# hmorimitsu/ptlflow

Measured on AMD Instinct MI355X. Metric: frame-pairs/sec, RAFT 32-iter 436x1024, higher is better.
Workload: dtype f32; 1 GPU; raft random-init (seeded), 436x1024 frame pairs, 32 iterations, fp32, batch 8/GPU, eval forward incl. encoders, mask head + convex upsample on every iteration as the reference; global_batch=8, parallelism=dp1 (independent replicas, no collectives)

## Files before the change

ptlflow_amd/csrc/pfk_wino.hip:

```cpp
#include "pfk_gemm.h"

using namespace pfkg;

namespace {

constexpr int WT = 32;
constexpr int WN = 64;
constexpr int WK = 8;
constexpr int UIMG = 16 * WN * WK;

typedef float f32x2 __attribute__((ext_vector_type(2)));
typedef __attribute__((address_space(3))) float lfloat;
typedef __attribute__((address_space(3))) f32x2 lf32x2;
typedef __attribute__((address_space(3))) f32x4 lf32x4;

struct WinoArgs {
  const float* src; int ld;
  unsigned src_bytes;
  int H, W;
  int tw, tpi;
  int ntiles;
  int nks;
  const float* weight; unsigned w_bytes;
  const float* bias;
  int cout;
  int ncb;
  int relu; float scale;
  float* out; int out_ld, out_coff;
  const float* res; int res_ld;
  int relu2;
};

__device__ __forceinline__ __amdgpu_buffer_rsrc_t rsrc_n(const void* p, unsigned bytes) {
  return __builtin_amdgcn_make_buffer_rsrc(const_cast<void*>(p), 0, (int)bytes, 0x00020000);
}

__device__ __forceinline__ void wino_load_v2(__amdgpu_buffer_rsrc_t rs, const unsigned (&voff)[16], int ks, int q, float (&d)[16]) {
  d[q] = __builtin_bit_cast(float, __builtin_amdgcn_raw_buffer_load_b32(rs, voff[q], ks * WK * 4, 0));
  d[q + 1] = __builtin_bit_cast(float, __builtin_amdgcn_raw_buffer_load_b32(rs, voff[q + 1], ks * WK * 4, 0));
}

__device__ __forceinline__ void wino_dma_u(__amdgpu_buffer_rsrc_t rw, lfloat* dst, unsigned wvoff, unsigned wk, int j) {
#if defined(__HIP_DEVICE_COMPILE__)
  __builtin_amdgcn_raw_ptr_buffer_load_lds(rw, (__attribute__((address_space(3))) void*)(dst + j * 1024), 16, wvoff, wk + j * 4096u, 0, 0);
#endif
}

__device__ __forceinline__ void wino_mfma(const lfloat* aV, const lfloat* aU, const lfloat* aU1, f32x4 (&acc)[16][2], bool more,
                                          __amdgpu_buffer_rsrc_t rw, lfloat* udst, unsigned wvoff, unsigned wk,
                                          __amdgpu_buffer_rsrc_t rs, const unsigned (&voff)[16], int ks, float (&d)[16]) {
  f32x2 va[2], u0[2], u1[2];
  va[0] = *(const lf32x2*)(aV);
  u0[0] = *(const lf32x2*)(aU);
  u1[0] = *(const lf32x2*)(aU1);
  __builtin_amdgcn_sched_barrier(0);
#pragma unroll
  for (int x = 0; x < 16; ++x) {
    const int c = x & 1, n = c ^ 1;
    if (x + 1 < 16) {
      va[n] = *(const lf32x2*)(aV + (x + 1) * WT * WK);
      u0[n] = *(const lf32x2*)(aU + (x + 1) * WN * WK);
      u1[n] = *(const lf32x2*)(aU1 + (x + 1) * WN * WK);
    }
    if (more) {
      if (x < 8) wino_dma_u(rw, udst, wvoff, wk, x);
      else wino_load_v2(rs, voff, ks, 2 * (x - 8), d);
    }
    __builtin_amdgcn_sched_barrier(0);
    acc[x][0] = __builtin_amdgcn_mfma_f32_16x16x4f32(va[c][0], u0[c][0], acc[x][0], 0, 0, 0);
    acc[x][1] = __builtin_amdgcn_mfma_f32_16x16x4f32(va[c][0], u1[c][0], acc[x][1], 0, 0, 0);
    acc[x][0] = __builtin_amdgcn_mfma_f32_16x16x4f32(va[c][1], u0[c][1], acc[x][0], 0, 0, 0);
    acc[x][1] = __builtin_amdgcn_mfma_f32_16x16x4f32(va[c][1], u1[c][1], acc[x][1], 0, 0, 0);
    __builtin_amdgcn_sched_barrier(0);
  }
}

template <bool RES>
__global__ __launch_bounds__(256, 2) void conv_gemm_wino_f32_kernel(const WinoArgs a) {
  __shared__ __attribute__((aligned(16))) float smem[2 * UIMG + 16 * WT * WK];
  lfloat* const sU = (lfloat*)smem;
  lfloat* const sV = sU + 2 * UIMG;

  const int tid = threadIdx.x, lane = tid & 63, wid = __builtin_amdgcn_readfirstlane(tid >> 6);
  const int cb = blockIdx.x % a.ncb;
  const int t0 = (blockIdx.x / a.ncb) * WT;

  const __amdgpu_buffer_rsrc_t rs = rsrc_n(a.src, a.src_bytes);
  const __amdgpu_buffer_rsrc_t rw = rsrc_n(a.weight, a.w_bytes);

  const int lt = tid >> 3, cc = tid & 7;
  unsigned voff[16];
  {
    const int g = t0 + lt;
    const bool tok = g < a.ntiles;
    const int b = g / a.tpi, r = g - b * a.tpi;
    const int ty = r / a.tw, tx = r - ty * a.tw;
#pragma unroll
    for (int i = 0; i < 4; ++i)
#pragma unroll
      for (int j = 0; j < 4; ++j) {
        const int y = 2 * ty - 1 + i, x = 2 * tx - 1 + j;
        const bool ok = tok && (unsigned)y < (unsigned)a.H && (unsigned)x < (unsigned)a.W;
        voff[i * 4 + j] = ok ? ((unsigned)((b * a.H + y) * a.W + x) * (unsigned)a.ld + (unsigned)cc) * 4u : OOB;
      }
  }
  const int vslot = ((cc & 3) * 2 + (cc >> 2)) ^ (((lt >> 2) & 3) * 2);
  lfloat* const vdst = sV + lt * WK + vslot;
  const unsigned wvoff = (unsigned)lane * 16u;
  const unsigned wbase = (unsigned)cb * (unsigned)a.nks * (UIMG * 4u) + (unsigned)wid * 1024u;
  lfloat* const udst = sU + wid * 256;

  float d[16];
  const int wt = wid & 1, wc = wid >> 1;
  const int rl = lane & 15, kq = lane >> 4;
  const lfloat* const aV = sV + (wt * 16 + rl) * WK + ((kq * 2) ^ (((rl >> 2) & 3) * 2));
  const lfloat* const aU = sU + (wc * 32 + rl) * WK + ((kq * 2) ^ (((rl >> 2) & 3) * 2));
  const lfloat* aU1 = aU + 16 * WK;
  asm volatile("" : "+v"(aU1));

  f32x4 acc[16][2];
#pragma unroll
  for (int x = 0; x < 16; ++x)
#pragma unroll
    for (int c = 0; c < 2; ++c) acc[x][c] = f32x4{0.f, 0.f, 0.f, 0.f};

#pragma unroll
  for (int j = 0; j < 8; ++j) {
    wino_dma_u(rw, udst, wvoff, wbase, j);
    wino_load_v2(rs, voff, 0, 2 * j, d);
  }
  for (int ks = 0; ks < a.nks; ++ks) {
    float t[16];
#pragma unroll
    for (int j = 0; j < 4; ++j) {
      t[0 * 4 + j] = d[0 * 4 + j] - d[2 * 4 + j];
      t[1 * 4 + j] = d[1 * 4 + j] + d[2 * 4 + j];
      t[2 * 4 + j] = d[2 * 4 + j] - d[1 * 4 + j];
      t[3 * 4 + j] = d[1 * 4 + j] - d[3 * 4 + j];
    }
#pragma unroll
    for (int i = 0; i < 4; ++i) {
      vdst[(i * 4 + 0) * WT * WK] = t[i * 4 + 0] - t[i * 4 + 2];
      vdst[(i * 4 + 1) * WT * WK] = t[i * 4 + 1] + t[i * 4 + 2];
      vdst[(i * 4 + 2) * WT * WK] = t[i * 4 + 2] - t[i * 4 + 1];
      vdst[(i * 4 + 3) * WT * WK] = t[i * 4 + 1] - t[i * 4 + 3];
    }
    asm volatile("s_waitcnt vmcnt(0) lgkmcnt(0)\n\ts_barrier" ::: "memory");
    const int ub = (ks & 1) * UIMG;
    wino_mfma(aV, aU + ub, aU1 + ub, acc, ks + 1 < a.nks, rw, udst + (UIMG - ub), wvoff, wbase + (unsigned)(ks + 1) * (UIMG * 4u), rs,
              voff, ks + 1, d);
    asm volatile("s_waitcnt lgkmcnt(0)\n\ts_barrier" ::: "memory");
  }

  typedef __attribute__((address_space(1))) float gfloat;
  gfloat* const outp = (gfloat*)a.out;
#pragma unroll
  for (int c = 0; c < 2; ++c) {
    const int n = cb * WN + wc * 32 + c * 16 + rl;
    const bool nok = n < a.cout;
    const float bias = (a.bias != nullptr && nok) ? a.bias[n] : 0.f;
#pragma unroll
    for (int r = 0; r < 4; ++r) {
      const int g = t0 + wt * 16 + kq * 4 + r;
      float m[16];
#pragma unroll
      for (int x = 0; x < 16; ++x) m[x] = acc[x][c][r];
      float s0[4], s1[4];
#pragma unroll
      for (int j = 0; j < 4; ++j) {
        s0[j] = m[0 * 4 + j] + m[1 * 4 + j] + m[2 * 4 + j];
        s1[j] = m[1 * 4 + j] - m[2 * 4 + j] - m[3 * 4 + j];
      }
      float y[4];
      y[0] = s0[0] + s0[1] + s0[2];
      y[1] = s0[1] - s0[2] - s0[3];
      y[2] = s1[0] + s1[1] + s1[2];
      y[3] = s1[1] - s1[2] - s1[3];
      if (!nok || g >= a.ntiles) continue;
      const int b = g / a.tpi, rr = g - b * a.tpi;
      const int ty = rr / a.tw, tx = rr - ty * a.tw;
#pragma unroll
      for (int e = 0; e < 4; ++e) {
        const int oy = 2 * ty + (e >> 1), ox = 2 * tx + (e & 1);
        if (oy >= a.H || ox >= a.W) continue;
        float v = y[e] + bias;
        if (a.relu) v = (v < 0.f) ? 0.f : v;
        v *= a.scale;
        const long long p = ((long long)b * a.H + oy) * a.W + ox;
        if constexpr (RES) {
          v = a.res[p * a.res_ld + n] + v;
          if (a.relu2) v = (v < 0.f) ? 0.f : v;
        }
        outp[p * a.out_ld + a.out_coff + n] = v;
      }
    }
  }
}

constexpr int WN1 = 128;
constexpr int VIMG1 = 8 * WT * WK;

struct Wino1dArgs {
  const float* src0; const float* src1;
  int ld0, ld1;
  unsigned bytes0, bytes1;
  int nks0, nks;
  int H, W;
  int L, nt;
  int ntiles;
  const float* weight; unsigned w_bytes;
  const float* bias;
  int cout, ncb;
  int relu; float scale;
  float* out; int out_ld, out_coff;
  const float* res; int res_ld;
  float* h; int h_ld;
  float* aux_z; float* aux_rh;
  int ch;
};

template <bool VERT>
__device__ __forceinline__ void wino1d_tile(const Wino1dArgs& a, int g, int& base, int& t) {
  if constexpr (VERT) {
    const int r = g / a.W, x = g - r * a.W, b = r / a.nt;
    t = r - b * a.nt;
    base = b * a.H * a.W + x;
  } else {
    const int line = g / a.nt;
    t = g - line * a.nt;
    base = line * a.W;
  }
}

__device__ __forceinline__ void wino1d_load_v(__amdgpu_buffer_rsrc_t rs0, __amdgpu_buffer_rsrc_t rs1, const unsigned (&voff0)[8],
                                              const unsigned (&voff1)[8], bool s1, int soff, int q, float (&d)[8]) {
  d[q] = s1 ? __builtin_bit_cast(float, __builtin_amdgcn_raw_buffer_load_b32(rs1, voff1[q], soff, 0))
            : __builtin_bit_cast(float, __builtin_amdgcn_raw_buffer_load_b32(rs0, voff0[q], soff, 0));
}

__device__ __forceinline__ void wino1d_mfma(const lfloat* aV, const lfloat* aU0, const lfloat* aU1, const lfloat* aU2, const lfloat* aU3,
                                            f32x4 (&acc)[8][4], bool more, __amdgpu_buffer_rsrc_t rw, lfloat* udst, unsigned wvoff,
                                            unsigned wk, __amdgpu_buffer_rsrc_t rs0, __amdgpu_buffer_rsrc_t rs1,
                                            const unsigned (&voff0)[8], const unsigned (&voff1)[8], bool s1, int soff, float (&d)[8]) {
  f32x2 va[2], u[2][4];
  va[0] = *(const lf32x2*)(aV);
  u[0][0] = *(const lf32x2*)(aU0);
  u[0][1] = *(const lf32x2*)(aU1);
  u[0][2] = *(const lf32x2*)(aU2);
  u[0][3] = *(const lf32x2*)(aU3);
  __builtin_amdgcn_sched_barrier(0);
#pragma unroll
  for (int x = 0; x < 8; ++x) {
    const int c = x & 1, n = c ^ 1;
    if (x + 1 < 8) {
      va[n] = *(const lf32x2*)(aV + (x + 1) * WT * WK);
      u[n][0] = *(const lf32x2*)(aU0 + (x + 1) * WN1 * WK);
      u[n][1] = *(const lf32x2*)(aU1 + (x + 1) * WN1 * WK);
      u[n][2] = *(const lf32x2*)(aU2 + (x + 1) * WN1 * WK);
      u[n][3] = *(const lf32x2*)(aU3 + (x + 1) * WN1 * WK);
    }
    if (more) {
      wino_dma_u(rw, udst, wvoff, wk, x);
      wino1d_load_v(rs0, rs1, voff0, voff1, s1, soff, x, d);
    }
    __builtin_amdgcn_sched_barrier(0);
#pragma unroll
    for (int s = 0; s < 2; ++s)
#pragma unroll
      for (int f = 0; f < 4; ++f) acc[x][f] = __builtin_amdgcn_mfma_f32_16x16x4f32(va[c][s], u[c][f][s], acc[x][f], 0, 0, 0);
    __builtin_amdgcn_sched_barrier(0);
  }
}

__device__ __forceinline__ void wino1d_at(const f32x4 (&acc)[8][4], int f, int r, float (&y)[4]) {
  const float p12 = acc[1][f][r] + acc[2][f][r], q12 = acc[1][f][r] - acc[2][f][r];
  const float p34 = acc[3][f][r] + acc[4][f][r], q34 = acc[3][f][r] - acc[4][f][r];
  const float p56 = acc[5][f][r] + acc[6][f][r], q56 = acc[5][f][r] - acc[6][f][r];
  y[0] = acc[0][f][r] + p12 + p34 + p56;
  y[1] = q12 + 2.f * q34 + 0.5f * q56;
// ... 209 lines not shown

int pfk_conv1d_wino_f32(const pfk_conv_desc* d, pfk_stream_t stream) {
  if (!d) return PFK_ERR_BAD_ARG;
  const bool vert = d->kh == 5 && d->kw == 1;
  if (!vert && !(d->kh == 1 && d->kw == 5)) return PFK_ERR_UNSUPPORTED;
  if (d->stride > 1 || d->num_src < 1 || d->num_src > 2 || d->relu_after_residual) return PFK_ERR_UNSUPPORTED;
  if (d->epilogue != PFK_EPI_LINEAR && d->epilogue != PFK_EPI_GRU_ZR && d->epilogue != PFK_EPI_GRU_Q) return PFK_ERR_UNSUPPORTED;
  if (d->cout_active > 0 && d->cout_active < d->cout) return PFK_ERR_UNSUPPORTED;
  if (d->epilogue == PFK_EPI_LINEAR && d->residual) return PFK_ERR_UNSUPPORTED;
  if (!d->weight || d->B <= 0 || d->H <= 0 || d->W <= 0 || d->cout <= 0) return PFK_ERR_BAD_ARG;
  const long long M = (long long)d->B * d->H * d->W;
  int ktot = 0;
  for (int i = 0; i < d->num_src; ++i) {
    const pfk_conv_src& s = d->src[i];
    if (!s.ptr || s.channels <= 0 || s.ld < s.channels) return PFK_ERR_BAD_ARG;
    if (s.channels & 7) return PFK_ERR_UNSUPPORTED;
    if (reinterpret_cast<uintptr_t>(s.ptr) & 3u) return PFK_ERR_ALIGNMENT;
    if (M * s.ld * 4 >= 0x7fffffffLL) return PFK_ERR_UNSUPPORTED;
    ktot += s.channels;
  }
  const int ch = d->epilogue == PFK_EPI_GRU_ZR ? d->cout / 2 : d->cout;
  if (d->epilogue == PFK_EPI_LINEAR) {
    if (!d->out || d->out_coff < 0 || d->out_ld < d->out_coff + d->cout) return PFK_ERR_BAD_ARG;
    if (reinterpret_cast<uintptr_t>(d->out) & 3u) return PFK_ERR_ALIGNMENT;
  } else {
    if (!d->h || !d->aux_z || d->h_ld < ch || (d->epilogue == PFK_EPI_GRU_ZR && (!d->aux_rh || (d->cout & 1))) || (ch & 3))
      return PFK_ERR_BAD_ARG;
    if (d->residual && d->residual_ld < d->cout) return PFK_ERR_BAD_ARG;
    if (!pfk_aligned16(d->h) || !pfk_aligned16(d->aux_z) || !pfk_aligned16(d->aux_rh) || !pfk_aligned16(d->residual) || (d->h_ld & 3) ||
        (d->residual && (d->residual_ld & 3)))
      return PFK_ERR_ALIGNMENT;
  }
  if (!pfk_aligned16(d->weight)) return PFK_ERR_ALIGNMENT;
  const long long wfloats = pfk_conv_wino1d_weight_floats(ktot, d->cout);
  if (wfloats * 4 >= 0x7fffffffLL) return PFK_ERR_UNSUPPORTED;
  Wino1dArgs a{};
  const pfk_conv_src& s0 = d->src[0];
  const pfk_conv_src& s1 = d->src[d->num_src - 1];
  a.src0 = s0.ptr; a.ld0 = s0.ld; a.bytes0 = (unsigned)(((M - 1) * s0.ld + s0.channels) * 4);
  a.src1 = s1.ptr; a.ld1 = s1.ld; a.bytes1 = (unsigned)(((M - 1) * s1.ld + s1.channels) * 4);
  a.nks0 = s0.channels / WK; a.nks = ktot / WK;
  a.H = d->H; a.W = d->W;
  a.L = vert ? d->H : d->W;
  a.nt = (a.L + 3) / 4;
  const long long ntiles = (long long)d->B * (vert ? d->W : d->H) * a.nt;
  a.ncb = (d->cout + WN1 - 1) / WN1;
  const long long nblk = (ntiles + WT - 1) / WT * a.ncb;
  if (nblk >= 0x7fffffffLL) return PFK_ERR_UNSUPPORTED;
  a.ntiles = (int)ntiles;
  a.weight = d->weight; a.w_bytes = (unsigned)(wfloats * 4);
  a.bias = d->bias;
  a.cout = d->cout;
  a.relu = d->relu ? 1 : 0; a.scale = d->scale;
  a.out = d->out; a.out_ld = d->out_ld; a.out_coff = d->out_coff;
  a.res = d->residual; a.res_ld = d->residual_ld;
  a.h = d->h; a.h_ld = d->h_ld; a.aux_z = d->aux_z; a.aux_rh = d->aux_rh; a.ch = ch;
  if (vert) wino1d_launch_epi<true>(a, d->epilogue, (unsigned)nblk, static_cast<hipStream_t>(stream));
  else wino1d_launch_epi<false>(a, d->epilogue, (unsigned)nblk, static_cast<hipStream_t>(stream));
  return pfk_launch_status();
}

long long pfk_conv_wino_weight_floats(int cin, int cout) {
  if (cin <= 0 || cout <= 0 || (cin & 31)) return PFK_ERR_BAD_ARG;
  return 16LL * cin * ((cout + WN - 1) / WN * WN);
}

static int wino_launch(const pfk_conv_desc* d, bool res, pfk_stream_t stream) {
  if (!d) return PFK_ERR_BAD_ARG;
  if (d->num_src != 1 || d->kh != 3 || d->kw != 3 || d->stride > 1 || d->epilogue != PFK_EPI_LINEAR)
    return PFK_ERR_UNSUPPORTED;
  if (!res && (d->residual || d->relu_after_residual)) return PFK_ERR_UNSUPPORTED;
  if (res && (!d->residual || d->residual_ld < d->cout || (reinterpret_cast<uintptr_t>(d->residual) & 3u))) return PFK_ERR_BAD_ARG;
  const pfk_conv_src& s = d->src[0];
  if (!s.ptr || !d->weight || !d->out || d->B <= 0 || d->H <= 0 || d->W <= 0 || d->cout <= 0 || s.channels <= 0 ||
      s.ld < s.channels || d->out_coff < 0 || d->out_ld < d->out_coff + d->cout)
    return PFK_ERR_BAD_ARG;
  if (s.channels & 31) return PFK_ERR_UNSUPPORTED;
  if (!pfk_aligned16(d->weight) || (reinterpret_cast<uintptr_t>(s.ptr) & 3u) || (reinterpret_cast<uintptr_t>(d->out) & 3u))
    return PFK_ERR_ALIGNMENT;
  const long long M = (long long)d->B * d->H * d->W;
  const long long src_bytes = ((M - 1) * s.ld + s.channels) * 4;
  const long long wfloats = pfk_conv_wino_weight_floats(s.channels, d->cout);
  if (M * s.ld * 4 >= 0x7fffffffLL || wfloats * 4 >= 0x7fffffffLL) return PFK_ERR_UNSUPPORTED;
  int ncb = (d->cout + WN - 1) / WN;
  if (d->cout_active > 0 && d->cout_active < d->cout) {
    if (d->cout_active & (WN - 1)) return PFK_ERR_UNSUPPORTED;
    ncb = d->cout_active / WN;
  }
  WinoArgs a{};
  a.src = s.ptr; a.ld = s.ld; a.src_bytes = (unsigned)src_bytes;
  a.H = d->H; a.W = d->W;
  a.tw = (d->W + 1) / 2;
  a.tpi = a.tw * ((d->H + 1) / 2);
  const long long ntiles = (long long)d->B * a.tpi;
  const long long nblk = (ntiles + WT - 1) / WT * ncb;
  if (nblk >= 0x7fffffffLL) return PFK_ERR_UNSUPPORTED;
  a.ntiles = (int)ntiles;
  a.nks = s.channels / WK;
  a.weight = d->weight; a.w_bytes = (unsigned)(wfloats * 4);
  a.bias = d->bias;
  a.cout = d->cout;
  a.ncb = ncb;
  a.relu = d->relu ? 1 : 0; a.scale = d->scale;
  a.out = d->out; a.out_ld = d->out_ld; a.out_coff = d->out_coff;
  if (res) {
    if (d->cout_active > 0 && d->cout_active < d->cout) return PFK_ERR_UNSUPPORTED;
    a.res = d->residual; a.res_ld = d->residual_ld; a.relu2 = d->relu_after_residual ? 1 : 0;
    hipLaunchKernelGGL(conv_gemm_wino_f32_kernel<true>, dim3((unsigned)nblk), dim3(256), 0, static_cast<hipStream_t>(stream), a);
  } else {
    hipLaunchKernelGGL(conv_gemm_wino_f32_kernel<false>, dim3((unsigned)nblk), dim3(256), 0, static_cast<hipStream_t>(stream), a);
  }
  return pfk_launch_status();
}

int pfk_conv2d_wino_f32(const pfk_conv_desc* d, pfk_stream_t stream) { return wino_launch(d, false, stream); }

int pfk_conv2d_wino_res_f32(const pfk_conv_desc* d, pfk_stream_t stream) { return wino_launch(d, true, stream); }



}
```

ptlflow_amd/update.py:

```python
from __future__ import annotations

from dataclasses import dataclass
from typing import Dict, List, Optional, Tuple

import torch

from . import load_native
from ._seam import WrappedModule, pixel_rows
from .packing import (pack_cin2_weight, pack_conv_weight, pack_flow_head_weight, pack_wino1d_weight, pack_wino_weight, permute_mask_head,
                      round_up, split_bf16_planes)

EPI_LINEAR, EPI_GRU_ZR, EPI_GRU_Q = 0, 1, 2


@dataclass(frozen=True)
class UpdateSpec:
    hidden: int
    context: int
    corr_channels: int
    c1: int
    c2: int
    f1: int
    f2: int
    enc_out: int
    gru_passes: Tuple[Tuple[int, int, str], ...]
    fh_hidden: int
    has_mask: bool
    aggregate: bool = False
    mask_channels: int = 576
    external_aggregate: bool = False

    @property
    def motion_channels(self) -> int:
        return self.enc_out + 2

    @property
    def x_channels(self) -> int:
        return self.context + self.motion_channels * (2 if self.aggregate else 1)

    @property
    def hx_channels(self) -> int:
        return round_up(self.hidden + self.x_channels, 4)


def basic_spec(corr_levels: int = 4, corr_radius: int = 4) -> UpdateSpec:
    return UpdateSpec(128, 128, corr_levels * (2 * corr_radius + 1) ** 2, 256, 192, 128, 64, 126,
                      ((1, 5, "1"), (5, 1, "2")), 256, True)


def gma_spec(corr_levels: int = 4, corr_radius: int = 4) -> UpdateSpec:
    return UpdateSpec(128, 128, corr_levels * (2 * corr_radius + 1) ** 2, 256, 192, 128, 64, 126,
                      ((1, 5, "1"), (5, 1, "2")), 256, True, True)


def ccmr_spec(corr_channels: int, mask_channels: int = 36) -> UpdateSpec:
    return UpdateSpec(128, 128, corr_channels, 256, 192, 128, 64, 126, ((1, 5, "1"), (5, 1, "2")), 256, True, True,
                      mask_channels, True)


def ms_raft_plus_spec(corr_channels: int, mask_channels: int = 36) -> UpdateSpec:
    return UpdateSpec(128, 128, corr_channels, 256, 192, 128, 64, 126, ((1, 5, "1"), (5, 1, "2")), 256, True, False,
                      mask_channels)


def small_spec(corr_levels: int = 4, corr_radius: int = 3) -> UpdateSpec:
    return UpdateSpec(96, 64, corr_levels * (2 * corr_radius + 1) ** 2, 96, 0, 64, 32, 80,
                      ((3, 3, ""),), 128, False)


WINO_MIN_WORK = 28160

WINO1D_MIN_PIXELS = 28160

SMALL_GRID_PIXELS = 28160

CONV_PRECISIONS = {"fp32": 0, "bf16": 1, "bf16x3": 2, "bf16x6": 3}


class UpdateEngine:

    def __init__(self, params: Dict[str, torch.Tensor], spec: UpdateSpec, device: torch.device,
                 conv_precision: str = "fp32", hoist_context: bool = True):
        load_native()
        self.hoist_context = bool(hoist_context)
        if conv_precision not in CONV_PRECISIONS:
            raise ValueError(f"conv_precision must be one of {sorted(CONV_PRECISIONS)}, got {conv_precision!r}")
        self.conv_precision = conv_precision
        self.nsplit = CONV_PRECISIONS[conv_precision]
        self.b16 = conv_precision == "bf16" and not spec.external_aggregate
        self.ops = torch.ops.pfk
        self.spec = spec
        self.device = device
        self._shape: Optional[Tuple[int, int, int]] = None
        self._fault_host: Optional[torch.Tensor] = None
        self._fault_event = None
        self.profile: Optional[Dict[str, list]] = None
        self.flops: Dict[str, float] = {}
        self.bytes: Dict[str, float] = {}
        self.winograd = True
        self.pack(params)

    def pack(self, P: Dict[str, torch.Tensor]) -> None:
        s, dev = self.spec, self.device

        def g(name):
            return P[name].detach().to(device=dev, dtype=torch.float32)

        def seg1(c):
            return [(0, c, round_up(c, 8 if self.b16 else 4))]

        def pk(weight, segments):
            if self.b16:
                return pack_conv_weight(weight, segments, kpad=64).to(torch.bfloat16).contiguous()
            if self.nsplit == 0:
                return pack_conv_weight(weight, segments)
            return split_bf16_planes(pack_conv_weight(weight, segments), self.nsplit)

        w: Dict[str, torch.Tensor] = {}
        real = s.hidden + s.x_channels
        self._real_cin = {"c1": s.corr_channels, "c2": s.c1, "f2": s.f1, "cv": (s.c2 if s.c2 else s.c1) + s.f2,
                          "fm": s.hidden, "mk": s.fh_hidden}
        for _, _, sfx in s.gru_passes:
            self._real_cin["zr" + sfx] = real - (s.context if self.hoist_context else 0)
            self._real_cin["q" + sfx] = real - (s.context if self.hoist_context else 0)
            self._real_cin["zrc" + sfx] = s.context
            self._real_cin["qc" + sfx] = s.context
        w["c1.w"] = pk(g("encoder.convc1.weight"), seg1(s.corr_channels))
        w["c1.b"] = g("encoder.convc1.bias").contiguous()
        if s.c2:
            w["c2.w"] = pk(g("encoder.convc2.weight"), seg1(s.c1))
            w["c2.b"] = g("encoder.convc2.bias").contiguous()
        w["f1.w"] = pack_cin2_weight(g("encoder.convf1.weight"))
        w["f1.b"] = g("encoder.convf1.bias").contiguous()
        w["f2.w"] = pk(g("encoder.convf2.weight"), seg1(s.f1))
        w["f2.b"] = g("encoder.convf2.bias").contiguous()
        cf = (s.c2 if s.c2 else s.c1) + s.f2
        w["cv.w"] = pk(g("encoder.conv.weight"), seg1(cf))
        w["cv.b"] = g("encoder.conv.bias").contiguous()
        Ch = s.hidden
        hxc = round_up(s.hidden + s.x_channels, 8) if self.b16 else s.hx_channels
        real = Ch + s.x_channels
        for kh, kw, sfx in s.gru_passes:
            wz, wr, wq = (g(f"gru.conv{k}{sfx}.weight") for k in "zrq")
            bz, br, bq = (g(f"gru.conv{k}{sfx}.bias") for k in "zrq")
            if self.hoist_context:
                Ci = s.context
                rest = [(0, Ch, Ch), (Ch + Ci, real - Ch - Ci, hxc - Ch - Ci)]
                wzr = torch.cat([wz, wr], 0)
                w[f"zr{sfx}.w"] = pk(wzr, rest)
                w[f"q{sfx}.w"] = pk(wq, rest)
                if self.nsplit == 0 and not self.b16 and (kh, kw) in ((1, 5), (5, 1)) and rest[1][2] % 8 == 0 and Ch % 8 == 0:
                    w[f"zr{sfx}.w1d"] = pack_wino1d_weight(wzr, rest)
                    w[f"q{sfx}.w1d"] = pack_wino1d_weight(wq, rest)
                w[f"zrc{sfx}.w"] = pk(wzr, [(Ch, Ci, Ci)])
                w[f"zrc{sfx}.b"] = torch.cat([bz, br]).contiguous()
                w[f"qc{sfx}.w"] = pk(wq, [(Ch, Ci, Ci)])
                w[f"qc{sfx}.b"] = bq.contiguous()
                continue
            w[f"zr{sfx}.w"] = pk(torch.cat([wz, wr], 0), [(0, real, hxc)])
            w[f"zr{sfx}.b"] = torch.cat([bz, br]).contiguous()
            w[f"q{sfx}.w"] = pk(wq, [(0, Ch, Ch), (Ch, real - Ch, hxc - Ch)])
            w[f"q{sfx}.b"] = bq.contiguous()
        if s.has_mask:
            w["fm.w"] = pk(torch.cat([g("flow_head.conv1.weight"), g("mask.0.weight")], 0), seg1(Ch))
            w["fm.b"] = torch.cat([g("flow_head.conv1.bias"), g("mask.0.bias")]).contiguous()
            mask_hidden = g("mask.2.weight").shape[1]
            assert mask_hidden == g("mask.0.weight").shape[0], "mask.2 reads mask.0's output"
            w["mk.w"] = pk(g("mask.2.weight"), seg1(mask_hidden))
            w["mk.b"] = g("mask.2.bias").contiguous()
            if self.nsplit == 0 and s.mask_channels == 576 and mask_hidden % 32 == 0 and mask_hidden == s.fh_hidden:
                w["mku.w"], w["mku.b"] = permute_mask_head(pack_conv_weight(g("mask.2.weight"), seg1(mask_hidden)), w["mk.b"])
            elif self.b16 and s.mask_channels == 576 and mask_hidden % 64 == 0 and mask_hidden == s.fh_hidden:
                wp, bp = permute_mask_head(pack_conv_weight(g("mask.2.weight"), seg1(mask_hidden)), w["mk.b"])
                w["mku.w"], w["mku.b"] = wp.to(torch.bfloat16).contiguous(), bp
            w["fh.w"] = pk(g("flow_head.conv1.weight"), seg1(Ch))
            w["fh.b"] = g("flow_head.conv1.bias").contiguous()
            self._real_cin["fh"] = s.hidden
        else:
            w["fm.w"] = pk(g("flow_head.conv1.weight"), seg1(Ch))
            w["fm.b"] = g("flow_head.conv1.bias").contiguous()
        if s.aggregate and not s.external_aggregate:
            w["tv.w"] = pk(g("aggregator.to_v.weight"), seg1(s.motion_channels))
            w["tv.b"] = None
            self.gamma = float(P["aggregator.gamma"].detach().float().cpu().item())
            self._real_cin["tv"] = s.motion_channels
        if "flow_head.conv2.weight" in P:
            w["fh2.w"] = pack_flow_head_weight(g("flow_head.conv2.weight"))
            w["fh2.b"] = g("flow_head.conv2.bias").contiguous()
        if self.nsplit == 0 and not self.b16:
            fm = torch.cat([g("flow_head.conv1.weight"), g("mask.0.weight")], 0) if s.has_mask else g("flow_head.conv1.weight")
            wino = {"cv": g("encoder.conv.weight"), "fm": fm}
            if s.c2:
                wino["c2"] = g("encoder.convc2.weight")
            for key, wt in wino.items():
                if wt.shape[1] % 32 == 0 and tuple(wt.shape[2:]) == (3, 3):
                    w[key + ".ww"] = pack_wino_weight(wt)
        self.w = w

    def bind(self, B: int, H: int, W: int) -> None:
        if self._shape == (B, H, W):
            return
        s, dev = self.spec, self.device
        M = B * H * W
        z = lambda c: torch.zeros(M, c, device=dev, dtype=torch.float32)
        a = (lambda c: torch.zeros(M, c, device=dev, dtype=torch.bfloat16)) if self.b16 else z
        self.hx = z(s.hx_channels)
        self.hxb = a(round_up(s.hidden + s.x_channels, 8)) if self.b16 else None
        self.corr16 = a(round_up(s.corr_channels, 8)) if self.b16 else None
        self.cor1 = a(s.c1) if s.c2 else None
        self.corflo = a((s.c2 if s.c2 else s.c1) + s.f2)
        self.flo1 = a(s.f1)
        self.zbuf = a(s.hidden)
        self.rh = a(s.hidden)
        self.ctx = {("zr" + sfx): a(2 * s.hidden) for _, _, sfx in s.gru_passes} if self.hoist_context else {}
        if self.hoist_context:
            self.ctx.update({("q" + sfx): a(s.hidden) for _, _, sfx in s.gru_passes})
        self.fm = a(s.fh_hidden * (2 if s.has_mask else 1))
        self.mask = (a if s.mask_channels == 576 else z)(s.mask_channels) if s.has_mask else None
        self._scratch_c0 = torch.zeros(B, 2, H, W, device=dev, dtype=torch.float32)
        self._scratch_c1 = torch.zeros(B, 2, H, W, device=dev, dtype=torch.float32)
        self._delta = torch.zeros(B, 2, H, W, device=dev, dtype=torch.float32)
        if s.aggregate and not s.external_aggregate:
            N = H * W
            self.vbuf = a(s.motion_channels)
            if self.b16:
                self.vT = torch.zeros(B, s.motion_channels, round_up(round_up(N, 8), 64), device=dev, dtype=torch.bfloat16)
            else:
                self.vT = torch.zeros(B, s.motion_channels, round_up(N, 32), device=dev, dtype=torch.float32)
            self.attn = None
        self._empty = torch.empty(0, device=dev, dtype=torch.float32)
        nws = self.ops.conv_workspace_bytes()
        self.workspace = torch.zeros(nws, device=dev, dtype=torch.uint8)
        self.workspace_flow = torch.zeros(nws, device=dev, dtype=torch.uint8)
        self.workspace_mask = torch.zeros(nws, device=dev, dtype=torch.uint8)
        self._shape, self.pixels = (B, H, W), M

    def tic(self):
        ev = torch.cuda.Event(enable_timing=True)
        ev.record()
        return ev

    def toc(self, t0, key: str, flops: float, nbytes: Optional[float] = None) -> None:
        self.profile.setdefault(key, []).append((t0, self.tic()))
        self.flops[key] = flops
        if nbytes is not None:
            self.bytes[key] = nbytes

    def faults(self) -> int:
        off = self.ops.conv_workspace_fault_offset()
        return sum(int(ws[off: off + 4].view(torch.int32).item()) for ws in (self.workspace, self.workspace_flow, self.workspace_mask))

    def watch_faults(self) -> None:
        if self._fault_host is None:
            self._fault_host = torch.zeros(3, dtype=torch.int32).pin_memory()
            self._fault_event = None
        if self._fault_event is not None and self._fault_event.query():
            n = int(self._fault_host.sum())
            self._fault_event = None
            if n:
                for ws in (self.workspace, self.workspace_flow, self.workspace_mask):
                    ws.zero_()
                raise RuntimeError(f"libpfk: {n} stream-K fix-up(s) timed out in an earlier forward (its affected tiles are NaN); "
                                   "the workspace has been re-initialised")
        if self._fault_event is None and not torch.cuda.is_current_stream_capturing():
            off = self.ops.conv_workspace_fault_offset()
            for i, ws in enumerate((self.workspace, self.workspace_flow, self.workspace_mask)):
                self._fault_host[i: i + 1].copy_(ws[off: off + 4].view(torch.int32), non_blocking=True)
            self._fault_event = torch.cuda.Event()
            self._fault_event.record()

    @property
    def act(self):
        return self.hxb if self.b16 else self.hx

# ... 54 lines not shown
        B, H, W = self._shape
        N = H * W
        o = s.hidden + s.context
        mc = s.motion_channels
        if self.b16:
            hxb = self.hxb.view(B, N, self.hxb.shape[1])
            self._conv([self.hxb[:, o: o + mc]], 1, 1, "tv", mc, relu=False, out=self.vbuf)
            self.vT[:, :, :N].copy_(self.vbuf.view(B, N, mc).transpose(1, 2))
            t0 = self.tic() if self.profile is not None else None
            self.ops.conv2d_b16([self.attn], 1, H, W, 1, 1, self.vT, None, mc, EPI_LINEAR, False, self.gamma,
                                hxb[:, :, o + mc: o + 2 * mc], None, None, None, None, hxb[:, :, o: o + mc])
            if t0 is not None:
                self.toc(t0, "ag", 2.0 * B * N * N * mc)
            return
        mf = self.hx[:, o: o + mc]
        self._conv([mf], 1, 1, "tv", mc, relu=False, out=self.vbuf)
        self.ops.pm_to_cm(self.vbuf, self.vT)
        if self.nsplit == 0 and B > 1:
            for b0 in range(0, B, 4):
                bs = list(range(b0, min(B, b0 + 4)))
                rows = [slice(b * N, (b + 1) * N) for b in bs]
                t0 = self.tic() if self.profile is not None else None
                self.ops.conv2d_group([self.attn[b] for b in bs], 1, H, W, [1] * len(bs), [self.vT[b] for b in bs],
                                      [self._empty] * len(bs), [0] * len(bs), [self.gamma] * len(bs),
                                      [self.hx[r, o + mc: o + 2 * mc] for r in rows], [self.hx[r, o: o + mc] for r in rows])
                if t0 is not None:
                    self.toc(t0, "ag", 2.0 * len(bs) * N * N * mc)
            return
        for b in range(B):
            rows = slice(b * N, (b + 1) * N)
            src = self.attn[b]
            t0 = self.tic() if self.profile is not None else None
            vt = self.vT[b] if self.nsplit == 0 else split_bf16_planes(self.vT[b], self.nsplit)
            self.ops.conv2d([src], 1, H, W, 1, 1, vt, None, mc, EPI_LINEAR, False, self.gamma,
                            self.hx[rows, o + mc: o + 2 * mc], None, None, None, self.workspace, self.hx[rows, o: o + mc])
            if t0 is not None:
                self.toc(t0, "ag", 2.0 * N * N * mc)

    def load_state(self, net: torch.Tensor, inp: torch.Tensor) -> None:
        B, H, W = self._shape
        for src, dst in ((net, self.h_view), (inp, self.inp_view)):
            src = src.float()
            if src.is_contiguous():
                self.ops.nchw_to_pm(src, dst)
            else:
                dst.view(B, H, W, dst.shape[1]).copy_(src.permute(0, 2, 3, 1))
        self.state_changed()
        self.prepare_context()

    def prepare_context(self) -> None:
        if not self.hoist_context:
            return
        Ch, Ci = self.spec.hidden, self.spec.context
        inp = self.act[:, Ch: Ch + Ci]
        for kh, kw, sfx in self.spec.gru_passes:
            self._conv([inp], kh, kw, "zrc" + sfx, 2 * Ch, relu=False, out=self.ctx["zr" + sfx])
            self._conv([inp], kh, kw, "qc" + sfx, Ch, relu=False, out=self.ctx["q" + sfx])

    def _conv(self, srcs: List[torch.Tensor], kh, kw, key, cout, relu=True, scale=1.0, out=None,
              epi=EPI_LINEAR, h=None, z=None, rh=None, workspace=True, residual=None, cout_active=0, cout_split=0):
        B, H, W = self._shape
        t0 = self.tic() if self.profile is not None else None
        ws = self.workspace if workspace is True else (workspace if isinstance(workspace, torch.Tensor) else None)
        if self._use_wino1d(key, B * H * W):
            self.ops.conv2d_wino1d(srcs, B, H, W, kh, kw, self.w[key + ".w1d"], self.w.get(key + ".b"), cout, epi, relu, scale, out,
                                   h, z, rh, residual)
        elif self._use_wino(key, B * H * W, cout):
            self.ops.conv2d_wino(srcs[0], B, H, W, self.w[key + ".ww"], self.w.get(key + ".b"), cout, relu, scale, out, cout_active)
        elif self.b16:
            hb = self.hxb[:, : self.spec.hidden] if epi != EPI_LINEAR else None
            self.ops.conv2d_b16(srcs, B, H, W, kh, kw, self.w[key + ".w"], self.w.get(key + ".b"), cout, epi, relu, scale,
                                out, h if epi == EPI_GRU_Q else None, hb, z, rh, residual)
        else:
            self.ops.conv2d(srcs, B, H, W, kh, kw, self.w[key + ".w"], self.w.get(key + ".b"), cout, epi, relu, scale,
                            out, h, z, rh, ws, residual, 1, False, cout_active, cout_split)
        if t0 is not None:
            cin = self._real_cin[key]
            if cout_active:
                key, cout = key + "_half", cout_active
            self.toc(t0, key, 2.0 * B * H * W * cout * kh * kw * cin,
                     (2.0 if self.b16 else 4.0) * (B * H * W * (cin + cout) + cout * kh * kw * cin))

    def _use_wino(self, key: str, pixels: int, cout: int) -> bool:
        return self.winograd and pixels * ((cout + 63) // 64) >= WINO_MIN_WORK and (key + ".ww") in self.w

    def _use_wino1d(self, key: str, pixels: int) -> bool:
        return self.winograd and pixels >= WINO1D_MIN_PIXELS and (key + ".w1d") in self.w

    def motion(self, corr_pm: torch.Tensor) -> None:
        self.motion_corr(corr_pm)
        self.motion_flow()
        self.motion_join()

    def motion_corr(self, corr_pm: torch.Tensor) -> None:
        s = self.spec
        if s.c2:
            self._conv([corr_pm], 1, 1, "c1", s.c1, out=self.cor1)
            self._conv([self.cor1], 3, 3, "c2", s.c2, out=self.corflo[:, : s.c2])
        else:
            self._conv([corr_pm], 1, 1, "c1", s.c1, out=self.corflo[:, : s.c1])

    def motion_flow(self, branch: bool = False) -> None:
        s = self.spec
        B, H, W = self._shape
        cor_c = s.c2 if s.c2 else s.c1
        self.ops.conv_cin2(self.flow_view, self.w["f1.w"], self.w["f1.b"], self.flo1, B, H, W, 7, True)
        self._conv([self.flo1], 3, 3, "f2", s.f2, out=self.corflo[:, cor_c: cor_c + s.f2],
                   workspace=self.workspace_flow if branch else True)

    @property
    def can_group(self) -> bool:
        return self.nsplit == 0 and not self.b16

    @property
    def wants_grouped_motion(self) -> bool:
        return self.can_group and self.pixels < SMALL_GRID_PIXELS

    def motion_grouped(self, corr_pm: torch.Tensor, prev_mask: bool = False) -> None:
        s = self.spec
        B, H, W = self._shape
        self.ops.conv_cin2(self.flow_view, self.w["f1.w"], self.w["f1.b"], self.flo1, B, H, W, 7, True)
        cor_c = s.c2 if s.c2 else s.c1
        srcs = [corr_pm, self.flo1]
        ks = [1, 3]
        keys = ["c1", "f2"]
        relu, scale = [1, 1], [1.0, 1.0]
        outs = [self.cor1 if s.c2 else self.corflo[:, : s.c1], self.corflo[:, cor_c: cor_c + s.f2]]
        if prev_mask:
            srcs.append(self.fm[:, s.fh_hidden:]); ks.append(1); keys.append("mk"); relu.append(0); scale.append(0.25); outs.append(self.mask)
        t0 = self.tic() if self.profile is not None else None
        self.ops.conv2d_group(srcs, B, H, W, ks, [self.w[k + ".w"] for k in keys],
                              [self.w[k + ".b"] for k in keys], relu, scale, outs, [])
        if t0 is not None:
            M = B * H * W
            self.toc(t0, "+".join(keys), sum(2.0 * M * o.shape[1] * k * k * self._real_cin[kk] for o, k, kk in zip(outs, ks, keys)),
                     sum(4.0 * (M * (self._real_cin[kk] + o.shape[1]) + o.shape[1] * k * k * self._real_cin[kk])
                         for o, k, kk in zip(outs, ks, keys)))
        if s.c2:
            self._conv([self.cor1], 3, 3, "c2", s.c2, out=self.corflo[:, : s.c2])
        self.motion_join()

    def motion_join(self) -> None:
        s = self.spec
        o = s.hidden + s.context
        self._conv([self.corflo], 3, 3, "cv", s.enc_out, out=self.act[:, o: o + s.enc_out])

    @property
    def motion_view(self):
        s = self.spec
        o = s.hidden + s.context
        return self.hx[:, o: o + s.motion_channels]

    @property
    def aggregate_view(self):
        s = self.spec
        o = s.hidden + s.context + s.motion_channels
        return self.hx[:, o: o + s.motion_channels]

    def gru(self) -> None:
        s = self.spec
        Ch = s.hidden
        act = self.act
        if self.hoist_context:
            rest = act[:, Ch + s.context:]
            for kh, kw, sfx in s.gru_passes:
                self._conv([act[:, :Ch], rest], kh, kw, "zr" + sfx, 2 * Ch, epi=EPI_GRU_ZR, h=self.h_view, z=self.zbuf, rh=self.rh,
                           residual=self.ctx["zr" + sfx])
                self._conv([self.rh, rest], kh, kw, "q" + sfx, Ch, epi=EPI_GRU_Q, h=self.h_view, z=self.zbuf,
                           residual=self.ctx["q" + sfx])
            return
        for kh, kw, sfx in s.gru_passes:
            self._conv([act], kh, kw, "zr" + sfx, 2 * Ch, epi=EPI_GRU_ZR, h=self.h_view, z=self.zbuf, rh=self.rh)
            self._conv([self.rh, act[:, Ch:]], kh, kw, "q" + sfx, Ch, epi=EPI_GRU_Q, h=self.h_view, z=self.zbuf)

    def motion_and_gru(self, corr_pm: torch.Tensor, grouped: bool = False, prev_mask: bool = False) -> None:
        s = self.spec
        if grouped:
            self.motion_grouped(corr_pm, prev_mask)
        else:
            self.motion(corr_pm)
        if s.aggregate:
            if s.external_aggregate:
                raise RuntimeError("this block's aggregate slot is filled by the caller: use motion(), aggregate_view, gru()")
            if self.attn is None:
                raise RuntimeError("GMA update block needs set_attention() before the first iteration")
            self._aggregate()
        self.gru()

    def heads(self, coords0: torch.Tensor, coords1: torch.Tensor, delta_out: Optional[torch.Tensor],
              want_mask: bool = True, write_flow: bool = True, mask_conv2: bool = True) -> None:
        s = self.spec
        self.heads_conv1(want_mask)
        self.flow_delta(coords0, coords1, delta_out, write_flow)
        if s.has_mask and want_mask and mask_conv2:
            self.mask_head()

    def heads_conv1(self, want_mask: bool = True) -> None:
        s = self.spec
        if s.has_mask and self.nsplit == 0 and s.fh_hidden % 64 == 0:
            self._conv([self.h_view], 3, 3, "fm", 2 * s.fh_hidden, out=self.fm, cout_active=0 if want_mask else s.fh_hidden,
                       cout_split=s.fh_hidden)
        elif s.has_mask and not want_mask and (self.b16 or self.pixels >= SMALL_GRID_PIXELS):
            self._conv([self.act[:, : s.hidden]], 3, 3, "fh", s.fh_hidden, out=self.fm[:, : s.fh_hidden])
        else:
            self._conv([self.act[:, : s.hidden]], 3, 3, "fm", s.fh_hidden * (2 if s.has_mask else 1), out=self.fm)

    def flow_delta(self, coords0: torch.Tensor, coords1: torch.Tensor, delta_out: Optional[torch.Tensor] = None,
                   write_flow: bool = True) -> None:
        s = self.spec
        if self.b16:
            o = s.hidden + s.context + s.enc_out
            self.ops.flow_delta(self.fm[:, : s.fh_hidden], self.w["fh2.w"], self.w["fh2.b"], coords0, coords1, delta_out,
                                self.flow_view if write_flow else None, self.hxb[:, o: o + 2] if write_flow else None)
            return
        self.ops.flow_delta(self.fm[:, : s.fh_hidden], self.w["fh2.w"], self.w["fh2.b"], coords0, coords1, delta_out,
                            self.flow_view if write_flow else None)

    def mask_head(self, side_stream: bool = False) -> None:
        s = self.spec
        self._conv([self.fm[:, s.fh_hidden:]], 1, 1, "mk", s.mask_channels, relu=False, scale=0.25, out=self.mask,
                   workspace=self.workspace_mask if side_stream else True)

# ... 143 lines not shown
```

Measured before the change: 116.1 frame-pairs/s.

## Stage Winograd epilogue through LDS for vectorized stores; route f2 conv to Winograd

After: 123.8 frame-pairs/s, median of 6. 6.7% higher.

```diff
diff --git a/ptlflow_amd/csrc/pfk_wino.hip b/ptlflow_amd/csrc/pfk_wino.hip
--- a/ptlflow_amd/csrc/pfk_wino.hip
+++ b/ptlflow_amd/csrc/pfk_wino.hip
@@ -27,9 +27,15 @@
   int ncb;
   int relu; float scale;
   float* out; int out_ld, out_coff;
+  unsigned out_bytes;
   const float* res; int res_ld;
+  unsigned res_bytes;
   int relu2;
+  int vec;
 };
+
+constexpr unsigned T_OK = 0x80000000u, T_ROW2 = 0x40000000u, T_COL2 = 0x20000000u, T_PIX = 0x1fffffffu;
+constexpr int ESZ = 64 * 32 + 4 * 16;
 
 __device__ __forceinline__ __amdgpu_buffer_rsrc_t rsrc_n(const void* p, unsigned bytes) {
   return __builtin_amdgcn_make_buffer_rsrc(const_cast<void*>(p), 0, (int)bytes, 0x00020000);
@@ -75,6 +81,66 @@
   }
 }
 
+typedef __attribute__((address_space(3))) unsigned lunsigned;
+typedef unsigned int u32x4v __attribute__((__vector_size__(16)));
+
+template <bool RES, bool VEC>
+__device__ __forceinline__ void wino_epi_request(const WinoArgs& a, const lunsigned* tT, int n0, unsigned (&oo)[8], f32x4 (&r4)[8]) {
+  unsigned ro[8];
+#pragma unroll
+  for (int i = 0; i < 8; ++i) {
+    oo[i] = tT[2 * i] + (unsigned)(a.out_coff + n0) * 4u;
+    if constexpr (RES) ro[i] = tT[4 * WT + 2 * i] + (unsigned)n0 * 4u;
+  }
+  if constexpr (RES) {
+    const __amdgpu_buffer_rsrc_t rr = rsrc_n(a.res, a.res_bytes);
+#pragma unroll
+    for (int i = 0; i < 8; ++i) {
+      if constexpr (VEC) {
+        r4[i] = __builtin_bit_cast(f32x4, __builtin_amdgcn_raw_buffer_load_b128(rr, ro[i], 0, 0));
+      } else {
+#pragma unroll
+        for (int j = 0; j < 4; ++j)
+          r4[i][j] = __builtin_bit_cast(float, __builtin_amdgcn_raw_buffer_load_b32(rr, n0 + j < a.cout ? ro[i] + 4u * j : OOB, 0, 0));
+      }
+    }
+  }
+}
+
+template <bool RES, bool VEC>
+__device__ __forceinline__ void wino_epi_store(const WinoArgs& a, const lfloat* rE, int n0, const unsigned (&oo)[8], const f32x4 (&r4)[8]) {
+  const __amdgpu_buffer_rsrc_t ro = rsrc_n(a.out, a.out_bytes);
+  const __amdgpu_buffer_rsrc_t rbias = rsrc_n(a.bias, a.bias != nullptr ? (unsigned)a.cout * 4u : 0u);
+  float bias4[4];
+#pragma unroll
+  for (int j = 0; j < 4; ++j) bias4[j] = __builtin_bit_cast(float, __builtin_amdgcn_raw_buffer_load_b32(rbias, (unsigned)(n0 + j) * 4u, 0, 0));
+  const float lo = a.relu ? 0.f : -__builtin_inff(), lo2 = a.relu2 ? 0.f : -__builtin_inff();
+#pragma unroll
+  for (int i = 0; i < 8; ++i) {
+    const f32x4 y = *(const lf32x4*)(rE + i * 256 + (i >> 1) * 16);
+    float v[4];
+#pragma unroll
+    for (int j = 0; j < 4; ++j) {
+      float t = y[j] + bias4[j];
+      t = (t < lo) ? lo : t;
+      if constexpr (RES) {
+        t = __builtin_fmaf(t, a.scale, r4[i][j]);
+        t = (t < lo2) ? lo2 : t;
+      } else {
+        t *= a.scale;
+      }
+      v[j] = t;
+    }
+    if constexpr (VEC) {
+      __builtin_amdgcn_raw_buffer_store_b128(__builtin_bit_cast(u32x4v, (f32x4{v[0], v[1], v[2], v[3]})), ro, oo[i], 0, 0);
+    } else {
+#pragma unroll
+      for (int j = 0; j < 4; ++j)
+        __builtin_amdgcn_raw_buffer_store_b32(__builtin_bit_cast(unsigned, v[j]), ro, n0 + j < a.cout ? oo[i] + 4u * j : OOB, 0, 0);
+    }
+  }
+}
+
 template <bool RES>
 __global__ __launch_bounds__(256, 2) void conv_gemm_wino_f32_kernel(const WinoArgs a) {
   __shared__ __attribute__((aligned(16))) float smem[2 * UIMG + 16 * WT * WK];
@@ -90,11 +156,13 @@
 
   const int lt = tid >> 3, cc = tid & 7;
   unsigned voff[16];
+  unsigned tinfo;
   {
     const int g = t0 + lt;
     const bool tok = g < a.ntiles;
     const int b = g / a.tpi, r = g - b * a.tpi;
     const int ty = r / a.tw, tx = r - ty * a.tw;
+    tinfo = tok ? (T_OK | (2 * ty + 1 < a.H ? T_ROW2 : 0u) | (2 * tx + 1 < a.W ? T_COL2 : 0u) | (unsigned)((b * a.H + 2 * ty) * a.W + 2 * tx)) : 0u;
 #pragma unroll
     for (int i = 0; i < 4; ++i)
 #pragma unroll
@@ -152,49 +220,55 @@
     asm volatile("s_waitcnt lgkmcnt(0)\n\ts_barrier" ::: "memory");
   }
 
-  typedef __attribute__((address_space(1))) float gfloat;
-  gfloat* const outp = (gfloat*)a.out;
-#pragma unroll
-  for (int c = 0; c < 2; ++c) {
-    const int n = cb * WN + wc * 32 + c * 16 + rl;
-    const bool nok = n < a.cout;
-    const float bias = (a.bias != nullptr && nok) ? a.bias[n] : 0.f;
-#pragma unroll
-    for (int r = 0; r < 4; ++r) {
-      const int g = t0 + wt * 16 + kq * 4 + r;
-      float m[16];
-#pragma unroll
-      for (int x = 0; x < 16; ++x) m[x] = acc[x][c][r];
-      float s0[4], s1[4];
-#pragma unroll
-      for (int j = 0; j < 4; ++j) {
-        s0[j] = m[0 * 4 + j] + m[1 * 4 + j] + m[2 * 4 + j];
-        s1[j] = m[1 * 4 + j] - m[2 * 4 + j] - m[3 * 4 + j];
-      }
-      float y[4];
-      y[0] = s0[0] + s0[1] + s0[2];
-      y[1] = s0[1] - s0[2] - s0[3];
-      y[2] = s1[0] + s1[1] + s1[2];
-      y[3] = s1[1] - s1[2] - s1[3];
-      if (!nok || g >= a.ntiles) continue;
-      const int b = g / a.tpi, rr = g - b * a.tpi;
-      const int ty = rr / a.tw, tx = rr - ty * a.tw;
-#pragma unroll
-      for (int e = 0; e < 4; ++e) {
-        const int oy = 2 * ty + (e >> 1), ox = 2 * tx + (e & 1);
-        if (oy >= a.H || ox >= a.W) continue;
-        float v = y[e] + bias;
-        if (a.relu) v = (v < 0.f) ? 0.f : v;
-        v *= a.scale;
-        const long long p = ((long long)b * a.H + oy) * a.W + ox;
-        if constexpr (RES) {
-          v = a.res[p * a.res_ld + n] + v;
-          if (a.relu2) v = (v < 0.f) ? 0.f : v;
+  lfloat* const sE = (lfloat*)smem + wid * ESZ;
+  lunsigned* const sT = (lunsigned*)((lfloat*)smem + 4 * ESZ);
+  static_assert(4 * ESZ + 8 * WT <= 2 * UIMG + 16 * WT * WK, "parking areas and offset table must fit into the loop's LDS");
+  {
+    const unsigned need = T_OK | ((cc & 2) ? T_ROW2 : 0u) | ((cc & 1) ? T_COL2 : 0u);
+    const bool ok = (tinfo & need) == need;
+    const unsigned pix = (tinfo & T_PIX) + (unsigned)(((cc >> 1) & 1) * a.W + (cc & 1));
+    const unsigned po = ok ? pix * (unsigned)a.out_ld * 4u : OOB;
+    const unsigned pr = ok ? pix * (unsigned)a.res_ld * 4u : OOB;
+    if (cc < 4) {
+      sT[cc * WT + lt] = po;
+      if constexpr (RES) sT[(4 + cc) * WT + lt] = pr;
+    }
+  }
+  asm volatile("s_waitcnt lgkmcnt(0)\n\ts_barrier" ::: "memory");
+
+  const int prow = lane >> 3, c4 = (lane & 7) * 4;
+  const int n0 = cb * WN + wc * 32 + c4;
+  const lunsigned* const tT = sT + (prow & 3) * WT + wt * 16 + (lane >> 5);
+  const bool vec = a.vec && cb * WN + wc * 32 + 32 <= a.cout;
+  unsigned oo[8];
+  f32x4 r4[8];
+  if (vec) wino_epi_request<RES, true>(a, tT, n0, oo, r4);
+  else wino_epi_request<RES, false>(a, tT, n0, oo, r4);
+
+  {
+    lfloat* const pE = sE + kq * (16 * 32 + 16) + rl;
+#pragma unroll
+    for (int c = 0; c < 2; ++c)
+#pragma unroll
+      for (int r = 0; r < 4; ++r) {
+        float m[16];
+#pragma unroll
+        for (int x = 0; x < 16; ++x) m[x] = acc[x][c][r];
+        float s0[4], s1[4];
+#pragma unroll
+        for (int j = 0; j < 4; ++j) {
+          s0[j] = m[0 * 4 + j] + m[1 * 4 + j] + m[2 * 4 + j];
+          s1[j] = m[1 * 4 + j] - m[2 * 4 + j] - m[3 * 4 + j];
         }
-        outp[p * a.out_ld + a.out_coff + n] = v;
-      }
-    }
-  }
+        pE[(r * 4 + 0) * 32 + c * 16] = s0[0] + s0[1] + s0[2];
+        pE[(r * 4 + 1) * 32 + c * 16] = s0[1] - s0[2] - s0[3];
+        pE[(r * 4 + 2) * 32 + c * 16] = s1[0] + s1[1] + s1[2];
+        pE[(r * 4 + 3) * 32 + c * 16] = s1[1] - s1[2] - s1[3];
+      }
+  }
+  const lfloat* const rE = sE + prow * 32 + c4;
+  if (vec) wino_epi_store<RES, true>(a, rE, n0, oo, r4);
+  else wino_epi_store<RES, false>(a, rE, n0, oo, r4);
 }
 
 constexpr int WN1 = 128;
@@ -570,6 +644,9 @@
   const long long src_bytes = ((M - 1) * s.ld + s.channels) * 4;
   const long long wfloats = pfk_conv_wino_weight_floats(s.channels, d->cout);
   if (M * s.ld * 4 >= 0x7fffffffLL || wfloats * 4 >= 0x7fffffffLL) return PFK_ERR_UNSUPPORTED;
+  const long long out_bytes = ((M - 1) * d->out_ld + d->out_coff + d->cout) * 4;
+  const long long res_bytes = res ? ((M - 1) * d->residual_ld + d->cout) * 4 : 0;
+  if (out_bytes >= 0x7fffffffLL || res_bytes >= 0x7fffffffLL) return PFK_ERR_UNSUPPORTED;
   int ncb = (d->cout + WN - 1) / WN;
   if (d->cout_active > 0 && d->cout_active < d->cout) {
     if (d->cout_active & (WN - 1)) return PFK_ERR_UNSUPPORTED;
@@ -590,10 +667,11 @@
   a.cout = d->cout;
   a.ncb = ncb;
   a.relu = d->relu ? 1 : 0; a.scale = d->scale;
-  a.out = d->out; a.out_ld = d->out_ld; a.out_coff = d->out_coff;
+  a.out = d->out; a.out_ld = d->out_ld; a.out_coff = d->out_coff; a.out_bytes = (unsigned)out_bytes;
+  a.vec = pfk_aligned16(d->out + d->out_coff) && !(d->out_ld & 3) && (!res || (pfk_aligned16(d->residual) && !(d->residual_ld & 3)));
   if (res) {
     if (d->cout_active > 0 && d->cout_active < d->cout) return PFK_ERR_UNSUPPORTED;
-    a.res = d->residual; a.res_ld = d->residual_ld; a.relu2 = d->relu_after_residual ? 1 : 0;
+    a.res = d->residual; a.res_ld = d->residual_ld; a.res_bytes = (unsigned)res_bytes; a.relu2 = d->relu_after_residual ? 1 : 0;
     hipLaunchKernelGGL(conv_gemm_wino_f32_kernel<true>, dim3((unsigned)nblk), dim3(256), 0, static_cast<hipStream_t>(stream), a);
   } else {
     hipLaunchKernelGGL(conv_gemm_wino_f32_kernel<false>, dim3((unsigned)nblk), dim3(256), 0, static_cast<hipStream_t>(stream), a);
diff --git a/ptlflow_amd/update.py b/ptlflow_amd/update.py
--- a/ptlflow_amd/update.py
+++ b/ptlflow_amd/update.py
@@ -69,6 +69,8 @@
 
 
 WINO_MIN_WORK = 28160
+
+WINO_F2_MIN_PIXELS = 28160
 
 WINO1D_MIN_PIXELS = 28160
 
@@ -189,7 +191,7 @@
             w["fh2.b"] = g("flow_head.conv2.bias").contiguous()
         if self.nsplit == 0 and not self.b16:
             fm = torch.cat([g("flow_head.conv1.weight"), g("mask.0.weight")], 0) if s.has_mask else g("flow_head.conv1.weight")
-            wino = {"cv": g("encoder.conv.weight"), "fm": fm}
+            wino = {"cv": g("encoder.conv.weight"), "fm": fm, "f2": g("encoder.convf2.weight")}
             if s.c2:
                 wino["c2"] = g("encoder.convc2.weight")
             for key, wt in wino.items():
@@ -410,7 +412,11 @@
                      (2.0 if self.b16 else 4.0) * (B * H * W * (cin + cout) + cout * kh * kw * cin))
 
     def _use_wino(self, key: str, pixels: int, cout: int) -> bool:
-        return self.winograd and pixels * ((cout + 63) // 64) >= WINO_MIN_WORK and (key + ".ww") in self.w
+        if not self.winograd or (key + ".ww") not in self.w:
+            return False
+        if key == "f2":
+            return pixels >= WINO_F2_MIN_PIXELS
+        return pixels * ((cout + 63) // 64) >= WINO_MIN_WORK
 
     def _use_wino1d(self, key: str, pixels: int) -> bool:
         return self.winograd and pixels >= WINO1D_MIN_PIXELS and (key + ".w1d") in self.w
@@ -454,6 +460,9 @@
         keys = ["c1", "f2"]
         relu, scale = [1, 1], [1.0, 1.0]
         outs = [self.cor1 if s.c2 else self.corflo[:, : s.c1], self.corflo[:, cor_c: cor_c + s.f2]]
+        f2_alone = self._use_wino("f2", B * H * W, s.f2)
+        if f2_alone:
+            srcs, ks, keys, relu, scale, outs = srcs[:1], ks[:1], keys[:1], relu[:1], scale[:1], outs[:1]
         if prev_mask:
             srcs.append(self.fm[:, s.fh_hidden:]); ks.append(1); keys.append("mk"); relu.append(0); scale.append(0.25); outs.append(self.mask)
         t0 = self.tic() if self.profile is not None else None
@@ -466,6 +475,8 @@
                          for o, k, kk in zip(outs, ks, keys)))
         if s.c2:
             self._conv([self.cor1], 3, 3, "c2", s.c2, out=self.corflo[:, : s.c2])
+        if f2_alone:
+            self._conv([self.flo1], 3, 3, "f2", s.f2, out=self.corflo[:, cor_c: cor_c + s.f2])
         self.motion_join()
 
     def motion_join(self) -> None:
```
